# adri-romsor/iterative_inference_segm

Measured on AMD Instinct MI355X. Metric: refined images/s (FCN-8 + standard DAE, 10-step iterative inference, 224x224, 11 classes), higher is better.
Workload: dtype f32; 1 GPU; BASELINE configs[1]: FCN-8 + standard DAE (f64c1p2, pool4, trackind, skip), 224x224x3, batch 64/GPU, 10 steps, step 0.1, early stop off; per batch: pred_fcn_fn, val_fn, pred_dae_fn+val_fn, refine, val_fn; global_batch=64, parallelism=dp1

## Files before the change

include/iiseg.h:

```cpp
#ifndef IISEG_H
#define IISEG_H

#include <stdint.h>

#ifdef __cplusplus
extern "C" {
#endif

typedef enum iiseg_status {
    IISEG_OK = 0,
    IISEG_ERR_NULL = -1,
    IISEG_ERR_SHAPE = -2,
    IISEG_ERR_ALIGN = -3,
    IISEG_ERR_LAUNCH = -4,
    IISEG_ERR_UNSUPPORTED = -5
} iiseg_status;

const char* iiseg_strerror(int status);
const char* iiseg_last_hip_error(void);
int iiseg_abi_version(void);
const char* iiseg_target_arch(void);

int iiseg_profile_begin(int capacity);
int iiseg_profile_count(void);
// ... 40 lines not shown
int iiseg_conv_pool_f32(void* stream, const iiseg_conv_desc* d, const float* x1, const float* x2,
                        const float* pre, const float* pooled, const float* wp, const int32_t* ktab,
                        const float* bias, const float* add, float* out, float* pool_out);

int iiseg_conv_mask_supported(const iiseg_conv_desc* d);
int iiseg_conv_mask_f32(void* stream, const iiseg_conv_desc* d, const float* x1, const float* x2,
                        const float* pre, const float* pooled, const uint8_t* mask_in,
                        const float* wp, const int32_t* ktab, const float* bias, const float* add,
                        float* out, float* pool_out, uint8_t* mask_out);

int iiseg_conv_halo_seam(int on);
int64_t iiseg_conv_halo_seam_launches(void);

int iiseg_conv_bnrelu_supported(const iiseg_conv_desc* d);
int iiseg_conv_bnrelu_f32(void* stream, const iiseg_conv_desc* d, const float* x, int64_t x_bstride,
                          const float* beta, const float* gamma, const float* mean,
                          const float* inv_std, const float* wp, const int32_t* ktab,
                          const float* bias, float* out);

#define IISEG_WINO_INPUT 1u
#define IISEG_WINO_GEMM 2u
#define IISEG_WINO_OUTPUT 4u
#define IISEG_WINO_ALL 7u
#define IISEG_WINO_FUSED 8u
int iiseg_conv_wino_supported(const iiseg_conv_desc* d);
int64_t iiseg_conv_wino_weight_elems(const iiseg_conv_desc* d);
int64_t iiseg_conv_wino_workspace_elems(const iiseg_conv_desc* d);
int iiseg_conv_wino_pack_f32(void* stream, const iiseg_conv_desc* d, const float* w,
                             int64_t stride_o, int64_t stride_c, float* U);
int iiseg_conv_wino_f32(void* stream, const iiseg_conv_desc* d, const float* x1, const float* x2,
                        const float* pre, const float* pooled, const float* U, const float* bias,
                        const float* add, float* workspace, float* out, uint32_t stages);
int iiseg_conv_wino_input_wide(int on);
int iiseg_conv_wino_input_path(const iiseg_conv_desc* d, int mask_bytes);
int iiseg_conv_wino_pool_supported(const iiseg_conv_desc* d);
int iiseg_conv_wino_mask_f32(void* stream, const iiseg_conv_desc* d, const float* x1, const float* x2,
                             const float* pre, const float* pooled, const uint8_t* mask_in,
                             const float* U, const float* bias, const float* add, float* workspace,
                             float* out, float* pool_out, uint8_t* mask_out, uint32_t stages);

int iiseg_conv_wino_bf16_supported(const iiseg_conv_desc* d);
int64_t iiseg_conv_wino_bf16_weight_bytes(const iiseg_conv_desc* d);
int64_t iiseg_conv_wino_bf16_workspace_bytes(const iiseg_conv_desc* d);
int iiseg_conv_wino_bf16_pack(void* stream, const iiseg_conv_desc* d, const float* w,
                              int64_t stride_o, int64_t stride_c, void* U16);
int iiseg_conv_wino_bf16(void* stream, const iiseg_conv_desc* d, const float* x1, const float* x2,
                         const float* pre, const float* pooled, const void* U16, const float* bias,
                         const float* add, void* workspace, float* out, uint32_t stages);

int iiseg_conv_gemm_bf16_supported(const iiseg_conv_desc* d);
int64_t iiseg_conv_gemm_bf16_weight_bytes(const iiseg_conv_desc* d);
int64_t iiseg_conv_gemm_bf16_workspace_bytes(const iiseg_conv_desc* d);
int iiseg_conv_gemm_bf16_pack(void* stream, const iiseg_conv_desc* d, const float* w,
                              int64_t stride_o, int64_t stride_c, void* U16);
int iiseg_conv_gemm_bf16(void* stream, const iiseg_conv_desc* d, const float* x, const void* U16,
                         const float* bias, void* workspace, float* out);

int iiseg_conv_halo_bf16_supported(const iiseg_conv_desc* d);
int64_t iiseg_conv_halo_bf16_weight_bytes(const iiseg_conv_desc* d);
int iiseg_conv_halo_bf16_pack(void* stream, const iiseg_conv_desc* d, const float* w,
                              int64_t stride_o, int64_t stride_c, void* wp16);
int iiseg_conv_halo_bf16(void* stream, const iiseg_conv_desc* d, const float* x1, const float* x2,
                         const float* pre, const float* pooled, const void* wp16, const float* bias,
                         const float* add, float* out, float* pool_out, const uint8_t* mask_in,
                         uint8_t* mask_out);

// ... 336 lines not shown
```

iterative_inference_segm_amd/_lib.py:

```python
import ctypes as C
import os

HERE = os.path.dirname(os.path.abspath(__file__))
LIB_PATH = os.path.join(HERE, 'libiiseg_hip.so')

ABI_VERSION = 34

CONV_RELU = 1
CONV_UNPOOL = 2
CONV_X3 = 8
CONV_TRANSPOSED2 = 4
CONV_ZINS = 16


class ConvDesc(C.Structure):
    _fields_ = [(n, C.c_int32) for n in
                ('B', 'C1', 'C2', 'H', 'W', 'Cout', 'KH', 'KW', 'pad', 'dil',
                 'oy0', 'ox0', 'OH', 'OW', 'AH', 'AW', 'ay0', 'ax0')] + \
               [('flags', C.c_uint32), ('Kpad', C.c_int32), ('Mpad', C.c_int32),
                ('out_ctot', C.c_int32), ('out_c0', C.c_int32),
                ('out_H', C.c_int32), ('out_W', C.c_int32), ('out_y0', C.c_int32),
                ('out_x0', C.c_int32), ('tile_y0', C.c_int32), ('tile_x0', C.c_int32)]


# ... 43 lines not shown


_vp, _i32, _i64, _f32, _f64 = C.c_void_p, C.c_int32, C.c_int64, C.c_float, C.c_double

SIGNATURES = {
    'iiseg_strerror': (C.c_char_p, [C.c_int]),
    'iiseg_last_hip_error': (C.c_char_p, []),
    'iiseg_abi_version': (C.c_int, []),
    'iiseg_profile_begin': (C.c_int, [C.c_int]),
    'iiseg_profile_count': (C.c_int, []),
    'iiseg_profile_end': (C.c_int, [C.POINTER(C.c_float), C.c_int]),
    'iiseg_target_arch': (C.c_char_p, []),
    'iiseg_conv_ktab_entries': (C.c_int, [C.POINTER(ConvDesc)]),
    'iiseg_conv_plan': (C.c_int, [C.POINTER(ConvDesc)]),
    'iiseg_conv_pack_f32': (C.c_int, [_vp, C.POINTER(ConvDesc), _vp, _i64, _i64, _vp, _vp]),
    'iiseg_conv_f32': (C.c_int, [_vp, C.POINTER(ConvDesc)] + [_vp] * 9),
    'iiseg_conv_small_supported': (C.c_int, [C.POINTER(ConvDesc)]),
    'iiseg_conv_pool_supported': (C.c_int, [C.POINTER(ConvDesc)]),
    'iiseg_conv_direct_kernel': (C.c_int, [C.POINTER(ConvDesc), C.c_int, C.c_int, C.POINTER(C.c_int32)]),
    'iiseg_conv_pool_f32': (C.c_int, [_vp, C.POINTER(ConvDesc)] + [_vp] * 10),
    'iiseg_conv_halo_seam': (C.c_int, [C.c_int]),
    'iiseg_conv_halo_seam_launches': (_i64, []),
    'iiseg_conv_mask_supported': (C.c_int, [C.POINTER(ConvDesc)]),
    'iiseg_conv_mask_f32': (C.c_int, [_vp, C.POINTER(ConvDesc)] + [_vp] * 12),
    'iiseg_conv_bnrelu_supported': (C.c_int, [C.POINTER(ConvDesc)]),
    'iiseg_conv_bnrelu_f32': (C.c_int, [_vp, C.POINTER(ConvDesc), _vp, _i64] + [_vp] * 8),
    'iiseg_conv_wino_supported': (C.c_int, [C.POINTER(ConvDesc)]),
    'iiseg_conv_wino_weight_elems': (_i64, [C.POINTER(ConvDesc)]),
    'iiseg_conv_wino_workspace_elems': (_i64, [C.POINTER(ConvDesc)]),
    'iiseg_conv_wino_pack_f32': (C.c_int, [_vp, C.POINTER(ConvDesc), _vp, _i64, _i64, _vp]),
    'iiseg_conv_wino_f32': (C.c_int, [_vp, C.POINTER(ConvDesc)] + [_vp] * 9 + [C.c_uint32]),
    'iiseg_conv_wino_pool_supported': (C.c_int, [C.POINTER(ConvDesc)]),
    'iiseg_conv_wino_input_wide': (C.c_int, [C.c_int]),
    'iiseg_conv_wino_input_path': (C.c_int, [C.POINTER(ConvDesc), C.c_int]),
    'iiseg_conv_wino_mask_f32': (C.c_int, [_vp, C.POINTER(ConvDesc)] + [_vp] * 12 + [C.c_uint32]),
    'iiseg_conv_wino_bf16_supported': (C.c_int, [C.POINTER(ConvDesc)]),
    'iiseg_conv_wino_bf16_weight_bytes': (_i64, [C.POINTER(ConvDesc)]),
    'iiseg_conv_wino_bf16_workspace_bytes': (_i64, [C.POINTER(ConvDesc)]),
    'iiseg_conv_wino_bf16_pack': (C.c_int, [_vp, C.POINTER(ConvDesc), _vp, _i64, _i64, _vp]),
    'iiseg_conv_wino_bf16': (C.c_int, [_vp, C.POINTER(ConvDesc)] + [_vp] * 9 + [C.c_uint32]),
    'iiseg_conv_gemm_bf16_supported': (C.c_int, [C.POINTER(ConvDesc)]),
    'iiseg_conv_gemm_bf16_weight_bytes': (_i64, [C.POINTER(ConvDesc)]),
    'iiseg_conv_gemm_bf16_workspace_bytes': (_i64, [C.POINTER(ConvDesc)]),
    'iiseg_conv_gemm_bf16_pack': (C.c_int, [_vp, C.POINTER(ConvDesc), _vp, _i64, _i64, _vp]),
    'iiseg_conv_gemm_bf16': (C.c_int, [_vp, C.POINTER(ConvDesc)] + [_vp] * 5),
    'iiseg_conv_halo_bf16_supported': (C.c_int, [C.POINTER(ConvDesc)]),
    'iiseg_conv_halo_bf16_weight_bytes': (_i64, [C.POINTER(ConvDesc)]),
    'iiseg_conv_halo_bf16_pack': (C.c_int, [_vp, C.POINTER(ConvDesc), _vp, _i64, _i64, _vp]),
    'iiseg_conv_halo_bf16': (C.c_int, [_vp, C.POINTER(ConvDesc)] + [_vp] * 11),
    'iiseg_conv_wino_f64_supported': (C.c_int, [C.POINTER(ConvDesc)]),
    'iiseg_conv_wino_f64_weight_elems': (_i64, [C.POINTER(ConvDesc)]),
    'iiseg_conv_wino_f64_workspace_elems': (_i64, [C.POINTER(ConvDesc)]),
    'iiseg_conv_wino_pack_f64': (C.c_int, [_vp, C.POINTER(ConvDesc), _vp, _i64, _i64, _vp]),
    'iiseg_conv_wino_f64': (C.c_int, [_vp, C.POINTER(ConvDesc)] + [_vp] * 9),
    'iiseg_conv_c8_supported': (C.c_int, [C.POINTER(ConvDesc)]),
    'iiseg_conv_c8_is_flat': (C.c_int, [C.POINTER(ConvDesc)]),
    'iiseg_conv_c8_force_tiling': (C.c_int, [C.c_int, C.c_int, C.c_int]),
    'iiseg_conv_c8_tiling': (C.c_int, [C.POINTER(ConvDesc), C.c_int, C.POINTER(C.c_int32)]),
    'iiseg_conv_c8': (C.c_int, [_vp, C.POINTER(ConvDesc)] + [_vp] * 6 + [_i32, _vp, _i32, _vp, _vp]),
    'iiseg_conv_c8_slice': (C.c_int, [_vp, C.POINTER(ConvDesc), _vp, _i32] + [_vp] * 5 + [_i32, _vp, _i32, _vp, _vp]),
    'iiseg_unpool_c8': (C.c_int, [_vp] * 4 + [C.c_int] * 7),
    'iiseg_conv_c8_m16_supported': (C.c_int, [C.POINTER(ConvDesc)]),
    'iiseg_conv_c8_m16': (C.c_int, [_vp, C.POINTER(ConvDesc), _vp, _i32] + [_vp] * 6 + [_i32]),
    'iiseg_conv_c8_m16_workspace_bytes': (_i64, [C.POINTER(ConvDesc)]),
    'iiseg_conv_c8_m16_ws': (C.c_int, [_vp, C.POINTER(ConvDesc), _vp, _i32] + [_vp] * 6 + [_i32, _vp, _i64, _vp, _vp, _f64] + [_vp] * 4 + [_i32]),
    'iiseg_conv1x1_c8_weight_bytes': (_i64, [C.c_int, C.c_int]),
# ... 146 lines not shown
```

iterative_inference_segm_amd/csrc/conv_wino.hip:

```cpp
#include <hip/hip_runtime.h>
#include <stdint.h>
#include <stdlib.h>
#include <atomic>
#include <type_traits>
#include "iiseg.h"
#include "common.h"
#include "conv_common.h"

using namespace iiseg;

namespace {

struct WinoParams {
    const float* x1;
    const float* x2;
    const float* pre;
    const float* pooled;
    const uint8_t* mask_in;
    int h2, w2;
    const float* U;
    const float* bias;
    const float* add;
    float* V;
    float* M;
    float* out;
    int B, C1, C2, H, W;
    int Cout, pad;
    int oy0, ox0, OH, OW;
    int ty0, tx0, nty, ntx;
    int T, Tpad;
    int Kc, Mpad;
    int AH, AW, ay0, ax0;
    int relu;
    int out_ctot, out_c0, out_H, out_W, out_y0, out_x0;
    int n_ttiles, n_mtiles;
    float* pool;
    uint8_t* mask_out;
    int pool_H, pool_W;
};

__device__ __forceinline__ float pool4(float v00, float v01, float v10, float v11) {
    const float a = v00 > v01 ? v00 : v01;
    const float b = v10 > v11 ? v10 : v11;
    return a > b ? a : b;
}

__device__ __forceinline__ void pool_store(const WinoParams& p, int b, int co, int ay, int ax,
                                           float v00, float v01, float v10, float v11) {
    const float m = pool4(v00, v01, v10, v11);
    const size_t po = ((size_t)b * p.Cout + co) * p.pool_H * p.pool_W + (size_t)(ay >> 1) * p.pool_W + (ax >> 1);
    p.pool[po] = m;
    if (p.mask_out)
        p.mask_out[po] = (uint8_t)((v00 == m ? 1u : 0u) | (v01 == m ? 2u : 0u) |
                                   (v10 == m ? 4u : 0u) | (v11 == m ? 8u : 0u));
}

constexpr int RSRC_W3 = 0x00027000;

__device__ __forceinline__ __amdgpu_buffer_rsrc_t mk_rsrc(const float* base, int bytes) {
    return __builtin_amdgcn_make_buffer_rsrc((void*)base, 0, bytes, RSRC_W3);
}

__global__ void wino_weight_kernel(const float* __restrict__ w, int64_t so, int64_t sc,
                                   float* __restrict__ U, int Cin, int Cout, int Kc, int Mpad) {
    const int64_t n = (int64_t)Kc * Mpad;
    for (int64_t i = blockIdx.x * (int64_t)blockDim.x + threadIdx.x; i < n;
         i += (int64_t)gridDim.x * blockDim.x) {
        const int c = (int)(i / Mpad), co = (int)(i % Mpad);
        double g[3][3], t[4][3];
        const bool real = c < Cin && co < Cout;
#pragma unroll
        for (int a = 0; a < 3; ++a)
#pragma unroll
            for (int b = 0; b < 3; ++b) g[a][b] = real ? (double)w[co * so + c * sc + a * 3 + b] : 0.0;
#pragma unroll
        for (int b = 0; b < 3; ++b) {
            t[0][b] = g[0][b];
            t[1][b] = 0.5 * (g[0][b] + g[1][b] + g[2][b]);
            t[2][b] = 0.5 * (g[0][b] - g[1][b] + g[2][b]);
            t[3][b] = g[2][b];
        }
#pragma unroll
        for (int a = 0; a < 4; ++a) {
            const double u0 = t[a][0], u1 = 0.5 * (t[a][0] + t[a][1] + t[a][2]),
                         u2 = 0.5 * (t[a][0] - t[a][1] + t[a][2]), u3 = t[a][2];
            U[(int64_t)(a * 4 + 0) * n + i] = (float)u0;
            U[(int64_t)(a * 4 + 1) * n + i] = (float)u1;
            U[(int64_t)(a * 4 + 2) * n + i] = (float)u2;
            U[(int64_t)(a * 4 + 3) * n + i] = (float)u3;
        }
    }
}

constexpr int ICH = 4;
template <bool UNPOOL, int PY, int PX, bool MB = false>
// ... 351 lines not shown
                const float* Lb = L + lbase[j] + RB[i] * NC;
                const float2 alo = *reinterpret_cast<const float2*>(La);
                const float2 ahi = *reinterpret_cast<const float2*>(La + 2);
                const float2 blo = *reinterpret_cast<const float2*>(Lb);
                const float2 bhi = *reinterpret_cast<const float2*>(Lb + 2);
                const float da[4] = {alo.x, alo.y, ahi.x, ahi.y}, db[4] = {blo.x, blo.y, bhi.x, bhi.y};
                float e[4];
#pragma unroll
                for (int jj = 0; jj < 4; ++jj) e[jj] = i == 1 ? da[jj] + db[jj] : da[jj] - db[jj];
                o[0][j] = e[0] - e[2];
                o[1][j] = e[1] + e[2];
                o[2][j] = e[2] - e[1];
                o[3][j] = e[1] - e[3];
            }
            if (FULL || nv == 4) {
#pragma unroll
                for (int x = 0; x < 4; ++x)
                    *reinterpret_cast<float4*>(vo + (size_t)(i * 4 + x) * xis) =
                        make_float4(o[x][0], o[x][1], o[x][2], o[x][3]);
            } else {
#pragma unroll
                for (int x = 0; x < 4; ++x)
#pragma unroll
                    for (int j = 0; j < 3; ++j)
                        if (j < nv) vo[(size_t)(i * 4 + x) * xis + j] = o[x][j];
            }
        }
    }
    };
    if (tw0 + 4 * NT <= p.T) run(std::true_type{});
    else run(std::false_type{});
}

template <int BM, int BN, int WM, int WN, int NBUF, int BK = 16>
__global__ __launch_bounds__(WM * WN * 64, 2) void wino_gemm_kernel(const WinoParams p) {
    constexpr int NCH = BK / 2;
    constexpr int WTM = BM / WM, WTN = BN / WN;
    constexpr int TM = WTM / 32, TN = WTN / 32;
    constexpr int NW = WM * WN, NT = NW * 64;
    constexpr int AV = BK * BM / 4, BV = BK * BN / 4;
    constexpr int NA = NW == 8 ? 256 : NT;
    constexpr int APT = AV / NA, BPT = BV / 256;
    static_assert((NW == 4 || NW == 8) && AV % NA == 0 && BV % 256 == 0, "tile config");

    __shared__ __attribute__((aligned(16))) float As[NBUF][BK][BM];
    __shared__ __attribute__((aligned(16))) float Bs[NBUF][BK][BN];

    const int per_xi = p.n_ttiles * p.n_mtiles;
    int xi, tt, mt;
    {
        const int nb = gridDim.x, bid = blockIdx.x;
        const int q = nb / 8, r = nb % 8, xcd = bid % 8, l = bid / 8;
        const int v = (xcd < r ? xcd * (q + 1) : r * (q + 1) + (xcd - r) * q) + l;
        xi = v / per_xi;
        const int w = v - xi * per_xi;
        constexpr int GP = 8;
        const int gsize = GP * p.n_mtiles;
        const int g = w / gsize, rr = w % gsize;
        const int gp = min(GP, p.n_ttiles - g * GP);
        tt = g * GP + rr % gp;
        mt = rr / gp;
    }
    const int m0 = mt * BM, t0 = tt * BN;
    const int tid = threadIdx.x, lane = tid & 63, wave = tid >> 6;
    const int wm = wave / WN, wn = wave % WN;
    const int l31 = lane & 31, lh = lane >> 5;

    const __amdgpu_buffer_rsrc_t arsrc = mk_rsrc(p.U + (size_t)xi * p.Kc * p.Mpad, p.Kc * p.Mpad * 4);
    const __amdgpu_buffer_rsrc_t brsrc = mk_rsrc(p.V + (size_t)xi * p.Kc * p.Tpad, p.Kc * p.Tpad * 4);
    const bool bstager = NW == 4 || wave < 4;
    const bool astager = NW == 4 || wave >= 4;
    const int atid = NW == 8 ? tid - 256 : tid;
    const int awave = NW == 8 ? wave - 4 : wave;

#define WINO_STAGE(KT, BUF)                                                                        \
    {                                                                                              \
        if (astager)                                                                               \
            static_for<0, APT>([&](auto J) __attribute__((always_inline)) {                        \
                constexpr int j = decltype(J)::value;                                              \
                const int f = j * NA + atid;                                                       \
                const int row = f / (BM / 4), c4 = f % (BM / 4);                                   \
                __builtin_amdgcn_raw_ptr_buffer_load_lds(                                          \
                    arsrc,                                                                         \
                    (__attribute__((address_space(3))) void*)(&As[BUF][0][0] + (j * NA + awave * 64) * 4), \
                    16, (int)(4u * (unsigned)(((KT) * BK + row) * p.Mpad + m0 + c4 * 4)), 0, 0, 0); \
            });                                                                                    \
        if (bstager)                                                                               \
            static_for<0, BPT>([&](auto J) __attribute__((always_inline)) {                        \
                constexpr int j = decltype(J)::value;                                              \
                const int f = j * 256 + (tid & 255);                                               \
                const int row = f / (BN / 4), c4 = f % (BN / 4);                                   \
                __builtin_amdgcn_raw_ptr_buffer_load_lds(                                          \
                    brsrc,                                                                         \
                    (__attribute__((address_space(3))) void*)(&Bs[BUF][0][0] + (j * 256 + (wave & 3) * 64) * 4), \
                    16, (int)(4u * (unsigned)(((KT) * BK + row) * p.Tpad + t0 + c4 * 4)), 0, 0, 0); \
            });                                                                                    \
    }

    f32x16 acc[TM][TN];
#pragma unroll
    for (int i = 0; i < TM; ++i)
#pragma unroll
        for (int j = 0; j < TN; ++j)
#pragma unroll
            for (int r = 0; r < 16; ++r) acc[i][j][r] = 0.f;

    const int nkt = p.Kc / BK;
    constexpr int OPS_A = APT, OPS_B = BPT;
#define WINO_WAIT_ONE_STAGE_IN_FLIGHT()                                                            \
    {                                                                                              \
        if constexpr (NW == 8) {                                                                   \
            if (astager) asm volatile("s_waitcnt vmcnt(%0)" ::"n"(OPS_A) : "memory");              \
            else asm volatile("s_waitcnt vmcnt(%0)" ::"n"(OPS_B) : "memory");                      \
        } else {                                                                                   \
            asm volatile("s_waitcnt vmcnt(%0)" ::"n"(OPS_A + OPS_B) : "memory");                   \
        }                                                                                          \
    }
    WINO_STAGE(0, 0)
    if constexpr (NBUF == 3) {
        if (nkt > 1) {
            WINO_STAGE(1, 1)
            WINO_WAIT_ONE_STAGE_IN_FLIGHT()
        } else {
            asm volatile("s_waitcnt vmcnt(0)" ::: "memory");
        }
    } else {
        asm volatile("s_waitcnt vmcnt(0)" ::: "memory");
    }
    __syncthreads();

    int buf = 0;
    for (int kt = 0; kt < nkt; ++kt) {
        const bool more = kt + NBUF - 1 < nkt;
        int sbuf = buf + NBUF - 1;
        if (sbuf >= NBUF) sbuf -= NBUF;
        float a[2][TM], b[2][TN];
#pragma unroll
        for (int i = 0; i < TM; ++i) a[0][i] = As[buf][lh][wm * WTM + i * 32 + l31];
#pragma unroll
        for (int j = 0; j < TN; ++j) b[0][j] = Bs[buf][lh][wn * WTN + j * 32 + l31];
        static_for<0, NCH>([&](auto CH) __attribute__((always_inline)) {
            constexpr int ch = decltype(CH)::value;
            if constexpr (ch + 1 < NCH) {
                const int kk = (ch + 1) * 2 + lh;
#pragma unroll
                for (int i = 0; i < TM; ++i) a[(ch + 1) & 1][i] = As[buf][kk][wm * WTM + i * 32 + l31];
#pragma unroll
                for (int j = 0; j < TN; ++j) b[(ch + 1) & 1][j] = Bs[buf][kk][wn * WTN + j * 32 + l31];
            }
#pragma unroll
            for (int i = 0; i < TM; ++i)
#pragma unroll
                for (int j = 0; j < TN; ++j)
                    acc[i][j] = __builtin_amdgcn_mfma_f32_32x32x2f32(a[ch & 1][i], b[ch & 1][j],
                                                                     acc[i][j], 0, 0, 0);
            if constexpr (ch == 0) {
                if (more) WINO_STAGE(kt + NBUF - 1, sbuf)
            }
            __builtin_amdgcn_sched_barrier(0);
        });
        if (NBUF == 3 && more) {
            WINO_WAIT_ONE_STAGE_IN_FLIGHT()
        } else {
            asm volatile("s_waitcnt vmcnt(0)" ::: "memory");
        }
        __syncthreads();
        if (++buf == NBUF) buf = 0;
    }
#undef WINO_STAGE
#undef WINO_WAIT_ONE_STAGE_IN_FLIGHT

    float* Mx = p.M + (size_t)xi * p.Mpad * p.Tpad;
#pragma unroll
    for (int j = 0; j < TN; ++j) {
        const int t = t0 + wn * WTN + j * 32 + l31;
#pragma unroll
        for (int i = 0; i < TM; ++i)
#pragma unroll
            for (int r = 0; r < 16; ++r) {
                const int co = m0 + wm * WTM + i * 32 + (r & 3) + 8 * (r >> 2) + 4 * lh;
                Mx[(size_t)co * p.Tpad + t] = acc[i][j][r];
            }
    }
}

template <int BM, int BN, int WM, int WN, int BK, int MINW>
__global__ __launch_bounds__(WM * WN * 64, MINW) void wino_fused_kernel(const WinoParams p) {
    constexpr int NCH = BK / 2;
    constexpr int WTM = BM / WM, WTN = BN / WN;
    constexpr int TM = WTM / 32, TN = WTN / 32;
    constexpr int NT = WM * WN * 64;
    constexpr int AV = BK * BM / 4, BV = BK * BN / 4;
    constexpr int APT = AV / NT, BPT = BV / NT;
    static_assert(AV % NT == 0 && BV % NT == 0, "tile config");

    __shared__ __attribute__((aligned(16))) float As[2][BK][BM];
    __shared__ __attribute__((aligned(16))) float Bs[2][BK][BN];

    int tt, mt;
    tile_of_block(blockIdx.x, gridDim.x, p.n_ttiles, p.n_mtiles, tt, mt);
    const int m0 = mt * BM, t0 = tt * BN;
    const int tid = threadIdx.x, lane = tid & 63, wave = tid >> 6;
    const int wm = wave / WN, wn = wave % WN;
    const int l31 = lane & 31, lh = lane >> 5;
    const int nkt = p.Kc / BK;
    const size_t ustride = (size_t)p.Kc * p.Mpad, vstride = (size_t)p.Kc * p.Tpad;
    const int ubytes = p.Kc * p.Mpad * 4, vbytes = p.Kc * p.Tpad * 4;

#define WINO_STAGE(XI, KT, BUF)                                                                    \
    {                                                                                              \
        const __amdgpu_buffer_rsrc_t ar = mk_rsrc(p.U + (size_t)(XI) * ustride, ubytes);           \
        const __amdgpu_buffer_rsrc_t br = mk_rsrc(p.V + (size_t)(XI) * vstride, vbytes);           \
        static_for<0, APT>([&](auto J) __attribute__((always_inline)) {                            \
            constexpr int j = decltype(J)::value;                                                  \
            const int f = j * NT + tid;                                                            \
            const int row = f / (BM / 4), c4 = f % (BM / 4);                                       \
            __builtin_amdgcn_raw_ptr_buffer_load_lds(                                              \
                ar, (__attribute__((address_space(3))) void*)(&As[BUF][0][0] + (j * NT + wave * 64) * 4), \
                16, (int)(4u * (unsigned)(((KT) * BK + row) * p.Mpad + m0 + c4 * 4)), 0, 0, 0);    \
        });                                                                                        \
        static_for<0, BPT>([&](auto J) __attribute__((always_inline)) {                            \
            constexpr int j = decltype(J)::value;                                                  \
            const int f = j * NT + tid;                                                            \
            const int row = f / (BN / 4), c4 = f % (BN / 4);                                       \
            __builtin_amdgcn_raw_ptr_buffer_load_lds(                                              \
                br, (__attribute__((address_space(3))) void*)(&Bs[BUF][0][0] + (j * NT + wave * 64) * 4), \
                16, (int)(4u * (unsigned)(((KT) * BK + row) * p.Tpad + t0 + c4 * 4)), 0, 0, 0);    \
        });                                                                                        \
    }

    f32x16 acc[TM][TN], Y[4][TM][TN];
#pragma unroll
    for (int i = 0; i < TM; ++i)
#pragma unroll
        for (int j = 0; j < TN; ++j)
#pragma unroll
            for (int r = 0; r < 16; ++r) {
                acc[i][j][r] = 0.f;
                Y[0][i][j][r] = Y[1][i][j][r] = Y[2][i][j][r] = Y[3][i][j][r] = 0.f;
            }

    WINO_STAGE(0, 0, 0)
    asm volatile("s_waitcnt vmcnt(0)" ::: "memory");
    __syncthreads();

    int xi = 0, kt = 0;
    const int total = 16 * nkt;
    for (int s = 0; s < total; ++s) {
        const int buf = s & 1;
        int nxi = xi, nkt1 = kt + 1;
        if (nkt1 == nkt) { nkt1 = 0; ++nxi; }
        const bool more = s + 1 < total;
        float a[2][TM], b[2][TN];
#pragma unroll
        for (int i = 0; i < TM; ++i) a[0][i] = As[buf][lh][wm * WTM + i * 32 + l31];
#pragma unroll
        for (int j = 0; j < TN; ++j) b[0][j] = Bs[buf][lh][wn * WTN + j * 32 + l31];
        static_for<0, NCH>([&](auto CH) __attribute__((always_inline)) {
            constexpr int ch = decltype(CH)::value;
            if constexpr (ch + 1 < NCH) {
                const int kk = (ch + 1) * 2 + lh;
#pragma unroll
                for (int i = 0; i < TM; ++i) a[(ch + 1) & 1][i] = As[buf][kk][wm * WTM + i * 32 + l31];
#pragma unroll
                for (int j = 0; j < TN; ++j) b[(ch + 1) & 1][j] = Bs[buf][kk][wn * WTN + j * 32 + l31];
            }
#pragma unroll
            for (int i = 0; i < TM; ++i)
#pragma unroll
                for (int j = 0; j < TN; ++j)
                    acc[i][j] = __builtin_amdgcn_mfma_f32_32x32x2f32(a[ch & 1][i], b[ch & 1][j],
                                                                     acc[i][j], 0, 0, 0);
            if constexpr (ch == 0) {
                if (more) WINO_STAGE(nxi, nkt1, buf ^ 1)
            }
            __builtin_amdgcn_sched_barrier(0);
        });
        if (nkt1 == 0) {
            const int wi = xi >> 2, wj = xi & 3;
            const float r0 = wi < 3 ? 1.f : 0.f, r1 = wi == 0 ? 0.f : (wi == 1 ? 1.f : -1.f);
            const float c0 = wj < 3 ? 1.f : 0.f, c1 = wj == 0 ? 0.f : (wj == 1 ? 1.f : -1.f);
            const float k00 = r0 * c0, k01 = r0 * c1, k10 = r1 * c0, k11 = r1 * c1;
#define WINO_FOLD(Q, KQ)                                                                            \
            if ((KQ) != 0.f) {                                                                      \
                _Pragma("unroll") for (int i = 0; i < TM; ++i)                                      \
                _Pragma("unroll") for (int j = 0; j < TN; ++j)                                      \
                _Pragma("unroll") for (int r = 0; r < 16; ++r)                                      \
                    Y[Q][i][j][r] = fmaf((KQ), acc[i][j][r], Y[Q][i][j][r]);                        \
            }
            WINO_FOLD(0, k00)
            WINO_FOLD(1, k01)
            WINO_FOLD(2, k10)
            WINO_FOLD(3, k11)
#undef WINO_FOLD
#pragma unroll
            for (int i = 0; i < TM; ++i)
#pragma unroll
                for (int j = 0; j < TN; ++j)
#pragma unroll
                    for (int r = 0; r < 16; ++r) acc[i][j][r] = 0.f;
        }
        xi = nxi;
        kt = nkt1;
        asm volatile("s_waitcnt vmcnt(0)" ::: "memory");
        __syncthreads();
    }
#undef WINO_STAGE

    typedef float f32x2u __attribute__((ext_vector_type(2), aligned(4)));
    const int ntt = p.nty * p.ntx;
    const size_t OPL = (size_t)p.out_H * p.out_W, APL = (size_t)p.AH * p.AW;
    float* Lbias = &As[0][0][0];
    for (int f = tid; f < BM; f += NT) Lbias[f] = (p.bias && m0 + f < p.Cout) ? p.bias[m0 + f] : 0.f;
    __syncthreads();
    float bias_r[TM][16];
#pragma unroll
    for (int i = 0; i < TM; ++i)
#pragma unroll
        for (int r = 0; r < 16; ++r) bias_r[i][r] = Lbias[wm * WTM + i * 32 + (r & 3) + 8 * (r >> 2) + 4 * lh];
#pragma unroll
    for (int j = 0; j < TN; ++j) {
        const int t = t0 + wn * WTN + j * 32 + l31;
        if (t >= p.T) continue;
        const int b = t / ntt;
        const int rr = t - b * ntt;
        const int tyl = rr / p.ntx, txl = rr - tyl * p.ntx;
        const int wy = p.ty0 + 2 * tyl - p.oy0, wx = p.tx0 + 2 * txl - p.ox0;
        const bool rok[2] = {(unsigned)wy < (unsigned)p.OH, (unsigned)(wy + 1) < (unsigned)p.OH};
        const bool cok[2] = {(unsigned)wx < (unsigned)p.OW, (unsigned)(wx + 1) < (unsigned)p.OW};
        const bool pair = cok[0] && cok[1];
        const bool whole = p.pool && rok[1] && cok[1];
        float* ob = p.out ? p.out + ((size_t)b * p.out_ctot + p.out_c0) * OPL +
                                (ptrdiff_t)(p.out_y0 + wy) * p.out_W + p.out_x0 + wx
                          : nullptr;
        const float* ab = p.add ? p.add + (size_t)b * p.Cout * APL +
                                      (ptrdiff_t)(p.ay0 + wy) * p.AW + p.ax0 + wx
                                : nullptr;
#pragma unroll
        for (int i = 0; i < TM; ++i)
#pragma unroll
            for (int r = 0; r < 16; ++r) {
                const int co = m0 + wm * WTM + i * 32 + (r & 3) + 8 * (r >> 2) + 4 * lh;
                if (co >= p.Cout) continue;
                const float bias = bias_r[i][r];
// ... 134 lines not shown
        d->pad < 0 || d->OH <= 0 || d->OW <= 0 || d->oy0 < 0 || d->ox0 < 0)
        return IISEG_ERR_SHAPE;
    const int fullH = d->H + 2 * d->pad - 2, fullW = d->W + 2 * d->pad - 2;
    if (d->oy0 + d->OH > fullH || d->ox0 + d->OW > fullW) return IISEG_ERR_SHAPE;
    if ((d->C1 + d->C2) % 16) return IISEG_ERR_UNSUPPORTED;
    g.Kc = d->C1 + d->C2;
    g.bm = d->Cout > 128 ? 256 : (d->Cout > 64 ? 128 : 64);
    g.Mpad = round_up(d->Cout, g.bm);
    if ((d->tile_y0 | d->tile_x0) & ~1) return IISEG_ERR_SHAPE;
    g.ty0 = d->oy0 - ((d->oy0 - d->tile_y0) & 1);
    g.tx0 = d->ox0 - ((d->ox0 - d->tile_x0) & 1);
    g.nty = (d->oy0 + d->OH - g.ty0 + 1) >> 1;
    g.ntx = (d->ox0 + d->OW - g.tx0 + 1) >> 1;
    const int64_t T = (int64_t)d->B * g.nty * g.ntx;
    const int64_t Tpad = (T + 127) / 128 * 128;
    if (Tpad * g.Kc * 4 >= (int64_t)1 << 31 || (int64_t)g.Kc * g.Mpad * 4 >= (int64_t)1 << 31)
        return IISEG_ERR_UNSUPPORTED;
    g.T = (int)T;
    g.Tpad = (int)Tpad;
    return IISEG_OK;
}

std::atomic<int> g_input_wide{-1};

int input_wide_setting() {
    int v = g_input_wide.load();
    if (v < 0) {
        v = getenv("IISEG_WINO_INPUT_WIDE") ? (atoi(getenv("IISEG_WINO_INPUT_WIDE")) != 0) : 1;
        g_input_wide.store(v);
    }
    return v;
}

bool iw_fits(const WinoParams& p, int nt) {
    const int NC = 2 * p.ntx + 2;
    for (int t0 = 0; t0 < p.T; t0 += 4 * nt) {
        const int t1 = t0 + 4 * nt < p.T ? t0 + 4 * nt : p.T;
        if ((int64_t)iw_chunk(t0, t1, p.ntx, p.nty).NR * NC > (int64_t)IW_E * nt) return false;
    }
    return true;
}

int ilds_nt(const WinoParams& p);
constexpr int IW_NT = 256;

int iw_shape(const WinoParams& p, bool unpool, bool mb) {
    const int setting = input_wide_setting();
    if (!setting || (unpool && !mb)) return 0;
    if (setting != 2) {
        if (p.T < 4096) return 0;
        const int lnt = mb ? 0 : ilds_nt(p);
        if (lnt && (p.nty * p.ntx) % lnt == 0) return 0;
    }
    const int64_t HW = (int64_t)p.H * p.W, cmax = p.C1 > p.C2 ? p.C1 : p.C2;
    if (HW > (1 << IW_PBITS) || (int64_t)p.B * cmax * HW >= (int64_t)1 << 30) return 0;
    const int64_t waves1 = ((int64_t)p.T + 255) / 256 * p.Kc;
    int ch = 8;
    if (p.Kc % 32 == 0 && waves1 / 32 >= 2048) ch = 32;
    else if (waves1 / 16 >= 2048) ch = 16;
    return iw_fits(p, IW_NT) ? ch : 0;
}

int ilds_nt(const WinoParams& p) {
    static const int lds = getenv("IISEG_WINO_INPUT_LDS") ? atoi(getenv("IISEG_WINO_INPUT_LDS")) : 1;
    const int ntt = p.nty * p.ntx;
    int nt = 0;
// ... 54 lines not shown
                             int Tpad, const float* bias, const float* add, float* out) {
    WinoParams p = {};
    p.M = const_cast<float*>(M);
    p.bias = bias; p.add = add; p.out = out;
    p.B = d->B; p.Cout = d->Cout; p.pad = d->pad;
    p.oy0 = d->oy0; p.ox0 = d->ox0; p.OH = d->OH; p.OW = d->OW;
    p.ty0 = d->oy0 - ((d->oy0 - d->tile_y0) & 1);
    p.tx0 = d->ox0 - ((d->ox0 - d->tile_x0) & 1);
    p.nty = (d->oy0 + d->OH - p.ty0 + 1) >> 1;
    p.ntx = (d->ox0 + d->OW - p.tx0 + 1) >> 1;
    p.T = d->B * p.nty * p.ntx;
    p.Tpad = Tpad; p.Mpad = Mpad;
    p.AH = d->AH; p.AW = d->AW; p.ay0 = d->ay0; p.ax0 = d->ax0;
    p.relu = (d->flags & IISEG_CONV_RELU) ? 1 : 0;
    p.out_ctot = d->out_ctot > 0 ? d->out_ctot : d->Cout;
    p.out_c0 = d->out_ctot > 0 ? d->out_c0 : 0;
    p.out_H = d->out_H > 0 ? d->out_H : d->OH;
    p.out_W = d->out_H > 0 ? d->out_W : d->OW;
    p.out_y0 = d->out_H > 0 ? d->out_y0 : 0;
    p.out_x0 = d->out_H > 0 ? d->out_x0 : 0;
    IISEG_LAUNCH(wino_output_kernel, dim3((p.T + 255) / 256, (d->Cout + OCH - 1) / OCH),
                       dim3(256), 0, s, p);
    return iiseg_check_launch();
}

extern "C" int iiseg_conv_wino_supported(const iiseg_conv_desc* d) {
    WinoGeom g;
    return wino_geom(d, g) == IISEG_OK ? 1 : 0;
}

extern "C" int iiseg_conv_wino_input_wide(int on) {
    if (on >= 0) g_input_wide.store(on > 1 ? 2 : on);
    return input_wide_setting();
}

extern "C" int iiseg_conv_wino_input_path(const iiseg_conv_desc* d, int mask_bytes) {
    WinoGeom g;
    const int st = wino_geom(d, g);
    if (st) return st;
    WinoParams p = {};
    const bool unpool = (d->flags & IISEG_CONV_UNPOOL) != 0;
    if (mask_bytes && !unpool) return IISEG_ERR_UNSUPPORTED;
    p.B = d->B; p.C1 = d->C1; p.C2 = d->C2; p.H = d->H; p.W = d->W;
    p.nty = g.nty; p.ntx = g.ntx; p.T = g.T; p.Tpad = g.Tpad; p.Kc = g.Kc;
    if (iw_shape(p, unpool, mask_bytes != 0)) return 2;
    return ilds_nt(p) ? 1 : 0;
}

extern "C" int64_t iiseg_conv_wino_weight_elems(const iiseg_conv_desc* d) {
    WinoGeom g;
    if (wino_geom(d, g) != IISEG_OK) return 0;
    return (int64_t)16 * g.Kc * g.Mpad;
}

extern "C" int64_t iiseg_conv_wino_workspace_elems(const iiseg_conv_desc* d) {
    WinoGeom g;
    if (wino_geom(d, g) != IISEG_OK) return 0;
    return (int64_t)16 * g.Tpad * ((int64_t)g.Kc + g.Mpad);
}

extern "C" int iiseg_conv_wino_pack_f32(void* stream, const iiseg_conv_desc* d, const float* w,
                                        int64_t stride_o, int64_t stride_c, float* U) {
    WinoGeom g;
    const int st = wino_geom(d, g);
    if (st) return st;
    if (!w || !U) return IISEG_ERR_NULL;
// ... 48 lines not shown
    p.U = U;
    p.bias = bias;
    p.add = add;
    p.V = workspace;
    p.M = workspace + (size_t)16 * g.Kc * g.Tpad;
    p.out = out;
    p.B = d->B; p.C1 = d->C1; p.C2 = d->C2; p.H = d->H; p.W = d->W;
    p.Cout = d->Cout; p.pad = d->pad;
    p.oy0 = d->oy0; p.ox0 = d->ox0; p.OH = d->OH; p.OW = d->OW;
    p.ty0 = g.ty0; p.tx0 = g.tx0; p.nty = g.nty; p.ntx = g.ntx;
    p.T = g.T; p.Tpad = g.Tpad; p.Kc = g.Kc; p.Mpad = g.Mpad;
    p.AH = d->AH; p.AW = d->AW; p.ay0 = d->ay0; p.ax0 = d->ax0;
    if (add && (d->ay0 < 0 || d->ax0 < 0 || d->ay0 + d->OH > d->AH || d->ax0 + d->OW > d->AW))
        return IISEG_ERR_SHAPE;
    p.relu = (d->flags & IISEG_CONV_RELU) ? 1 : 0;
    p.out_ctot = d->out_ctot > 0 ? d->out_ctot : d->Cout;
    p.out_c0 = d->out_ctot > 0 ? d->out_c0 : 0;
    if (p.out_c0 < 0 || p.out_c0 + d->Cout > p.out_ctot) return IISEG_ERR_SHAPE;
    p.out_H = d->out_H > 0 ? d->out_H : d->OH;
    p.out_W = d->out_H > 0 ? d->out_W : d->OW;
    p.out_y0 = d->out_H > 0 ? d->out_y0 : 0;
    p.out_x0 = d->out_H > 0 ? d->out_x0 : 0;
    if (p.out_y0 < 0 || p.out_x0 < 0 || p.out_y0 + d->OH > p.out_H || p.out_x0 + d->OW > p.out_W)
        return IISEG_ERR_SHAPE;
    p.n_ttiles = g.Tpad / 128;
    p.n_mtiles = g.Mpad / g.bm;
    hipStream_t s = (hipStream_t)stream;
    const int tb = (g.T + 255) / 256;
    if (stages & IISEG_WINO_FUSED) {
        if (g.Kc % 32) return IISEG_ERR_UNSUPPORTED;
        if (stages & IISEG_WINO_INPUT)
            launch_wino_input(s, p, unpool);
        if (stages & IISEG_WINO_GEMM) {
            if (g.bm == 64) {
                p.n_mtiles = g.Mpad / 64;
                IISEG_LAUNCH((wino_fused_kernel<64, 128, 1, 4, 32, 2>),
                                   dim3(p.n_ttiles * p.n_mtiles), dim3(256), 0, s, p);
                return iiseg_check_launch();
            }
            p.n_mtiles = g.Mpad / 128;
            const int w0 = p.n_ttiles * p.n_mtiles, w2 = (g.Tpad / 64) * p.n_mtiles;
            const double cost0 = (w0 + 255) / 256, cost2 = 0.5 * 1.03 * ((w2 + 255) / 256);
            static const int bk64 = getenv("IISEG_WINO_FUSED_BK") ? atoi(getenv("IISEG_WINO_FUSED_BK")) == 64 : 0;
            const bool big = bk64 && g.Kc % 64 == 0;
            if (g.Kc <= 128 || cost2 < cost0) {
                p.n_ttiles = g.Tpad / 64;
                if (big)
                    IISEG_LAUNCH((wino_fused_kernel<128, 64, 2, 2, 64, 2>),
                                       dim3(p.n_ttiles * p.n_mtiles), dim3(256), 0, s, p);
                else
                IISEG_LAUNCH((wino_fused_kernel<128, 64, 2, 2, 32, 2>),
                                   dim3(p.n_ttiles * p.n_mtiles), dim3(256), 0, s, p);
            } else if (big)
                IISEG_LAUNCH((wino_fused_kernel<128, 128, 2, 4, 64, 2>),
                                   dim3(p.n_ttiles * p.n_mtiles), dim3(512), 0, s, p);
            else
            IISEG_LAUNCH((wino_fused_kernel<128, 128, 2, 4, 32, 2>),
                               dim3(p.n_ttiles * p.n_mtiles), dim3(512), 0, s, p);
        }
        return iiseg_check_launch();
    }
    if (stages & IISEG_WINO_INPUT)
        launch_wino_input(s, p, unpool);
    const int grid = 16 * p.n_ttiles * p.n_mtiles;
    if (stages & IISEG_WINO_GEMM) {
        static const int nbuf = getenv("IISEG_WINO_NBUF") ? atoi(getenv("IISEG_WINO_NBUF")) : 2;
        int bm = g.bm;
        if (bm == 64) {
            IISEG_LAUNCH((wino_gemm_kernel<64, 128, 1, 4, 2>), dim3(grid), dim3(256), 0, s, p);
            bm = 0;
        }
        if (bm == 256) {
            const int w256 = grid, w128 = 2 * grid;
            if (0.5 * 1.06 * ((w128 + 255) / 256) < (double)((w256 + 255) / 256)) bm = 128;
        }
        const int grid2 = bm ? 16 * p.n_ttiles * (g.Mpad / bm) : 0;
        if (bm) p.n_mtiles = g.Mpad / bm;
        static const int bk32 = getenv("IISEG_WINO_GEMM_BK") ? atoi(getenv("IISEG_WINO_GEMM_BK")) == 32 : 0;
        if (bm && bk32 && g.Kc % 32 == 0 && nbuf != 3) {
            if (bm == 256)
                IISEG_LAUNCH((wino_gemm_kernel<256, 128, 4, 2, 2, 32>), dim3(grid), dim3(512), 0, s, p);
            else
                IISEG_LAUNCH((wino_gemm_kernel<128, 128, 2, 2, 2, 32>), dim3(grid2), dim3(256), 0, s, p);
        } else
        if (bm == 0) {
        } else if (bm == 256 && nbuf == 3)
            IISEG_LAUNCH((wino_gemm_kernel<256, 128, 4, 2, 3>), dim3(grid), dim3(512), 0, s, p);
        else if (bm == 256)
            IISEG_LAUNCH((wino_gemm_kernel<256, 128, 4, 2, 2>), dim3(grid), dim3(512), 0, s, p);
        else if (nbuf == 3)
            IISEG_LAUNCH((wino_gemm_kernel<128, 128, 2, 2, 3>), dim3(grid2), dim3(256), 0, s, p);
        else
            IISEG_LAUNCH((wino_gemm_kernel<128, 128, 2, 2, 2>), dim3(grid2), dim3(256), 0, s, p);
    }
    if (stages & IISEG_WINO_OUTPUT)
        IISEG_LAUNCH(wino_output_kernel, dim3(tb, (d->Cout + OCH - 1) / OCH), dim3(256), 0, s,
                           p);
    return iiseg_check_launch();
}

extern "C" int iiseg_conv_wino_f32(void* stream, const iiseg_conv_desc* d, const float* x1,
                                   const float* x2, const float* pre, const float* pooled,
                                   const float* U, const float* bias,
                                   const float* add, float* workspace, float* out,
                                   uint32_t stages) {
    return wino_run(stream, d, x1, x2, pre, pooled, nullptr, U, bias, add, workspace, out, nullptr,
                    nullptr, stages);
}

extern "C" int iiseg_conv_wino_mask_f32(void* stream, const iiseg_conv_desc* d, const float* x1,
                                        const float* x2, const float* pre, const float* pooled,
                                        const uint8_t* mask_in, const float* U, const float* bias,
// ... 148 lines not shown
```

Baseline: 536.1 images/s.

## Add configurable three-deep LDS ring to fused Winograd GEMM with inline-asm DMA

Replaces the builtin buffer-load-to-LDS calls with inline-asm buffer_load_dwordx4 ... lds using precomputed per-thread offsets and scalar k-offsets, and swaps __syncthreads for raw s_barrier. Adds an optional 3-buffer ring to the fused Winograd kernel, with partial vmcnt waits so that two stages can be in flight. Ring depth is selectable via env or API, but defaults stay at 2, so by default only the address and barrier rewrite takes effect. The hand-written m0 manipulation and raw barriers risk ordering bugs and add extra register pressure.

Result: no change. 541.0 images/s, median of 6 (+0.9%).

```diff
diff --git a/include/iiseg.h b/include/iiseg.h
--- a/include/iiseg.h
+++ b/include/iiseg.h
@@ -96,6 +96,7 @@
                         const float* pre, const float* pooled, const float* U, const float* bias,
                         const float* add, float* workspace, float* out, uint32_t stages);
 int iiseg_conv_wino_input_wide(int on);
+int iiseg_conv_wino_ring_depth(int fused, int depth);
 int iiseg_conv_wino_input_path(const iiseg_conv_desc* d, int mask_bytes);
 int iiseg_conv_wino_pool_supported(const iiseg_conv_desc* d);
 int iiseg_conv_wino_mask_f32(void* stream, const iiseg_conv_desc* d, const float* x1, const float* x2,
diff --git a/iterative_inference_segm_amd/_lib.py b/iterative_inference_segm_amd/_lib.py
--- a/iterative_inference_segm_amd/_lib.py
+++ b/iterative_inference_segm_amd/_lib.py
@@ -99,6 +99,7 @@
     'iiseg_conv_wino_f32': (C.c_int, [_vp, C.POINTER(ConvDesc)] + [_vp] * 9 + [C.c_uint32]),
     'iiseg_conv_wino_pool_supported': (C.c_int, [C.POINTER(ConvDesc)]),
     'iiseg_conv_wino_input_wide': (C.c_int, [C.c_int]),
+    'iiseg_conv_wino_ring_depth': (C.c_int, [C.c_int, C.c_int]),
     'iiseg_conv_wino_input_path': (C.c_int, [C.POINTER(ConvDesc), C.c_int]),
     'iiseg_conv_wino_mask_f32': (C.c_int, [_vp, C.POINTER(ConvDesc)] + [_vp] * 12 + [C.c_uint32]),
     'iiseg_conv_wino_bf16_supported': (C.c_int, [C.POINTER(ConvDesc)]),
diff --git a/iterative_inference_segm_amd/csrc/conv_wino.hip b/iterative_inference_segm_amd/csrc/conv_wino.hip
--- a/iterative_inference_segm_amd/csrc/conv_wino.hip
+++ b/iterative_inference_segm_amd/csrc/conv_wino.hip
@@ -55,12 +55,6 @@
                                    (v10 == m ? 4u : 0u) | (v11 == m ? 8u : 0u));
 }
 
-constexpr int RSRC_W3 = 0x00027000;
-
-__device__ __forceinline__ __amdgpu_buffer_rsrc_t mk_rsrc(const float* base, int bytes) {
-    return __builtin_amdgcn_make_buffer_rsrc((void*)base, 0, bytes, RSRC_W3);
-}
-
 __global__ void wino_weight_kernel(const float* __restrict__ w, int64_t so, int64_t sc,
                                    float* __restrict__ U, int Cin, int Cout, int Kc, int Mpad) {
     const int64_t n = (int64_t)Kc * Mpad;
@@ -478,6 +472,17 @@
     else run(std::false_type{});
 }
 
+__device__ __forceinline__ void ring_barrier() { asm volatile("s_barrier" ::: "memory"); }
+
+__device__ __forceinline__ void ring_dma16(i32x4s rsrc, unsigned lds, unsigned voff, unsigned soff) {
+    unsigned keep;
+    asm volatile("s_nop 1\n\ts_mov_b32 %0, m0\n\ts_mov_b32 m0, %1\n\ts_nop 0\n\t"
+                 "buffer_load_dwordx4 %2, %3, %4 offen lds\n\ts_mov_b32 m0, %0"
+                 : "=&s"(keep)
+                 : "s"(lds), "v"(voff), "s"(rsrc), "s"(soff)
+                 : "memory");
+}
+
 template <int BM, int BN, int WM, int WN, int NBUF, int BK = 16>
 __global__ __launch_bounds__(WM * WN * 64, 2) void wino_gemm_kernel(const WinoParams p) {
     constexpr int NCH = BK / 2;
@@ -512,35 +517,44 @@
     const int wm = wave / WN, wn = wave % WN;
     const int l31 = lane & 31, lh = lane >> 5;
 
-    const __amdgpu_buffer_rsrc_t arsrc = mk_rsrc(p.U + (size_t)xi * p.Kc * p.Mpad, p.Kc * p.Mpad * 4);
-    const __amdgpu_buffer_rsrc_t brsrc = mk_rsrc(p.V + (size_t)xi * p.Kc * p.Tpad, p.Kc * p.Tpad * 4);
+    const i32x4s arsrc = mk_srsrc(p.U + (size_t)xi * p.Kc * p.Mpad, (unsigned)(p.Kc * p.Mpad * 4));
+    const i32x4s brsrc = mk_srsrc(p.V + (size_t)xi * p.Kc * p.Tpad, (unsigned)(p.Kc * p.Tpad * 4));
     const bool bstager = NW == 4 || wave < 4;
     const bool astager = NW == 4 || wave >= 4;
-    const int atid = NW == 8 ? tid - 256 : tid;
-    const int awave = NW == 8 ? wave - 4 : wave;
-
+    const int atid = NW == 8 ? (tid & 255) : tid;
+    const int awave = NW == 8 ? (wave & 3) : wave;
+
+    unsigned aoff[APT], boff[BPT];
+#pragma unroll
+    for (int j = 0; j < APT; ++j) {
+        const int f = j * NA + atid;
+        const int row = f / (BM / 4), c4 = f % (BM / 4);
+        aoff[j] = 4u * (unsigned)(row * p.Mpad + m0 + c4 * 4);
+    }
+#pragma unroll
+    for (int j = 0; j < BPT; ++j) {
+        const int f = j * 256 + (tid & 255);
+        const int row = f / (BN / 4), c4 = f % (BN / 4);
+        boff[j] = 4u * (unsigned)(row * p.Tpad + t0 + c4 * 4);
+    }
+    const unsigned a_lds = __builtin_amdgcn_readfirstlane(lds_addr(&As[0][0][0]) + (unsigned)awave * 1024u);
+    const unsigned b_lds = __builtin_amdgcn_readfirstlane(lds_addr(&Bs[0][0][0]) + (unsigned)(wave & 3) * 1024u);
 #define WINO_STAGE(KT, BUF)                                                                        \
     {                                                                                              \
-        if (astager)                                                                               \
+        if (astager) {                                                                             \
+            const unsigned so = __builtin_amdgcn_readfirstlane(4u * (unsigned)((KT) * BK * p.Mpad)); \
             static_for<0, APT>([&](auto J) __attribute__((always_inline)) {                        \
                 constexpr int j = decltype(J)::value;                                              \
-                const int f = j * NA + atid;                                                       \
-                const int row = f / (BM / 4), c4 = f % (BM / 4);                                   \
-                __builtin_amdgcn_raw_ptr_buffer_load_lds(                                          \
-                    arsrc,                                                                         \
-                    (__attribute__((address_space(3))) void*)(&As[BUF][0][0] + (j * NA + awave * 64) * 4), \
-                    16, (int)(4u * (unsigned)(((KT) * BK + row) * p.Mpad + m0 + c4 * 4)), 0, 0, 0); \
+                ring_dma16(arsrc, a_lds + (unsigned)(BUF) * (BK * BM * 4u) + j * NA * 16u, aoff[j], so); \
             });                                                                                    \
-        if (bstager)                                                                               \
+        }                                                                                          \
+        if (bstager) {                                                                             \
+            const unsigned so = __builtin_amdgcn_readfirstlane(4u * (unsigned)((KT) * BK * p.Tpad)); \
             static_for<0, BPT>([&](auto J) __attribute__((always_inline)) {                        \
                 constexpr int j = decltype(J)::value;                                              \
-                const int f = j * 256 + (tid & 255);                                               \
-                const int row = f / (BN / 4), c4 = f % (BN / 4);                                   \
-                __builtin_amdgcn_raw_ptr_buffer_load_lds(                                          \
-                    brsrc,                                                                         \
-                    (__attribute__((address_space(3))) void*)(&Bs[BUF][0][0] + (j * 256 + (wave & 3) * 64) * 4), \
-                    16, (int)(4u * (unsigned)(((KT) * BK + row) * p.Tpad + t0 + c4 * 4)), 0, 0, 0); \
+                ring_dma16(brsrc, b_lds + (unsigned)(BUF) * (BK * BN * 4u) + j * 256 * 16u, boff[j], so); \
             });                                                                                    \
+        }                                                                                          \
     }
 
     f32x16 acc[TM][TN];
@@ -573,7 +587,7 @@
     } else {
         asm volatile("s_waitcnt vmcnt(0)" ::: "memory");
     }
-    __syncthreads();
+    ring_barrier();
 
     int buf = 0;
     for (int kt = 0; kt < nkt; ++kt) {
@@ -610,7 +624,8 @@
         } else {
             asm volatile("s_waitcnt vmcnt(0)" ::: "memory");
         }
-        __syncthreads();
+        ring_barrier();
+        __builtin_amdgcn_sched_barrier(0);
         if (++buf == NBUF) buf = 0;
     }
 #undef WINO_STAGE
@@ -630,7 +645,7 @@
     }
 }
 
-template <int BM, int BN, int WM, int WN, int BK, int MINW>
+template <int BM, int BN, int WM, int WN, int BK, int MINW, int NBUF = 2>
 __global__ __launch_bounds__(WM * WN * 64, MINW) void wino_fused_kernel(const WinoParams p) {
     constexpr int NCH = BK / 2;
     constexpr int WTM = BM / WM, WTN = BN / WN;
@@ -639,9 +654,10 @@
     constexpr int AV = BK * BM / 4, BV = BK * BN / 4;
     constexpr int APT = AV / NT, BPT = BV / NT;
     static_assert(AV % NT == 0 && BV % NT == 0, "tile config");
-
-    __shared__ __attribute__((aligned(16))) float As[2][BK][BM];
-    __shared__ __attribute__((aligned(16))) float Bs[2][BK][BN];
+    static_assert(NBUF == 2 || NBUF == 3, "ring depth");
+
+    __shared__ __attribute__((aligned(16))) float As[NBUF][BK][BM];
+    __shared__ __attribute__((aligned(16))) float Bs[NBUF][BK][BN];
 
     int tt, mt;
     tile_of_block(blockIdx.x, gridDim.x, p.n_ttiles, p.n_mtiles, tt, mt);
@@ -653,25 +669,34 @@
     const size_t ustride = (size_t)p.Kc * p.Mpad, vstride = (size_t)p.Kc * p.Tpad;
     const int ubytes = p.Kc * p.Mpad * 4, vbytes = p.Kc * p.Tpad * 4;
 
+    unsigned aoff[APT], boff[BPT];
+#pragma unroll
+    for (int j = 0; j < APT; ++j) {
+        const int f = j * NT + tid;
+        const int row = f / (BM / 4), c4 = f % (BM / 4);
+        aoff[j] = 4u * (unsigned)(row * p.Mpad + m0 + c4 * 4);
+    }
+#pragma unroll
+    for (int j = 0; j < BPT; ++j) {
+        const int f = j * NT + tid;
+        const int row = f / (BN / 4), c4 = f % (BN / 4);
+        boff[j] = 4u * (unsigned)(row * p.Tpad + t0 + c4 * 4);
+    }
+    const unsigned a_lds = __builtin_amdgcn_readfirstlane(lds_addr(&As[0][0][0]) + (unsigned)wave * 1024u);
+    const unsigned b_lds = __builtin_amdgcn_readfirstlane(lds_addr(&Bs[0][0][0]) + (unsigned)wave * 1024u);
 #define WINO_STAGE(XI, KT, BUF)                                                                    \
     {                                                                                              \
-        const __amdgpu_buffer_rsrc_t ar = mk_rsrc(p.U + (size_t)(XI) * ustride, ubytes);           \
-        const __amdgpu_buffer_rsrc_t br = mk_rsrc(p.V + (size_t)(XI) * vstride, vbytes);           \
+        const i32x4s ar = mk_srsrc(p.U + (size_t)(XI) * ustride, (unsigned)ubytes);                \
+        const i32x4s br = mk_srsrc(p.V + (size_t)(XI) * vstride, (unsigned)vbytes);                \
+        const unsigned soa = __builtin_amdgcn_readfirstlane(4u * (unsigned)((KT) * BK * p.Mpad));  \
+        const unsigned sob = __builtin_amdgcn_readfirstlane(4u * (unsigned)((KT) * BK * p.Tpad));  \
         static_for<0, APT>([&](auto J) __attribute__((always_inline)) {                            \
             constexpr int j = decltype(J)::value;                                                  \
-            const int f = j * NT + tid;                                                            \
-            const int row = f / (BM / 4), c4 = f % (BM / 4);                                       \
-            __builtin_amdgcn_raw_ptr_buffer_load_lds(                                              \
-                ar, (__attribute__((address_space(3))) void*)(&As[BUF][0][0] + (j * NT + wave * 64) * 4), \
-                16, (int)(4u * (unsigned)(((KT) * BK + row) * p.Mpad + m0 + c4 * 4)), 0, 0, 0);    \
+            ring_dma16(ar, a_lds + (unsigned)(BUF) * (BK * BM * 4u) + j * NT * 16u, aoff[j], soa); \
         });                                                                                        \
         static_for<0, BPT>([&](auto J) __attribute__((always_inline)) {                            \
             constexpr int j = decltype(J)::value;                                                  \
-            const int f = j * NT + tid;                                                            \
-            const int row = f / (BN / 4), c4 = f % (BN / 4);                                       \
-            __builtin_amdgcn_raw_ptr_buffer_load_lds(                                              \
-                br, (__attribute__((address_space(3))) void*)(&Bs[BUF][0][0] + (j * NT + wave * 64) * 4), \
-                16, (int)(4u * (unsigned)(((KT) * BK + row) * p.Tpad + t0 + c4 * 4)), 0, 0, 0);    \
+            ring_dma16(br, b_lds + (unsigned)(BUF) * (BK * BN * 4u) + j * NT * 16u, boff[j], sob); \
         });                                                                                        \
     }
 
@@ -686,17 +711,28 @@
                 Y[0][i][j][r] = Y[1][i][j][r] = Y[2][i][j][r] = Y[3][i][j][r] = 0.f;
             }
 
+    constexpr int OPS = APT + BPT;
+    const int total = 16 * nkt;
+    int sxi = 0, skt = 0;
     WINO_STAGE(0, 0, 0)
-    asm volatile("s_waitcnt vmcnt(0)" ::: "memory");
-    __syncthreads();
+    if (++skt == nkt) { skt = 0; ++sxi; }
+    if constexpr (NBUF == 3) {
+        WINO_STAGE(sxi, skt, 1)
+        if (++skt == nkt) { skt = 0; ++sxi; }
+        asm volatile("s_waitcnt vmcnt(%0)" ::"n"(OPS) : "memory");
+    } else {
+        asm volatile("s_waitcnt vmcnt(0)" ::: "memory");
+    }
+    ring_barrier();
 
     int xi = 0, kt = 0;
-    const int total = 16 * nkt;
+    int buf = 0;
     for (int s = 0; s < total; ++s) {
-        const int buf = s & 1;
-        int nxi = xi, nkt1 = kt + 1;
-        if (nkt1 == nkt) { nkt1 = 0; ++nxi; }
-        const bool more = s + 1 < total;
+        int nkt1 = kt + 1;
+        if (nkt1 == nkt) nkt1 = 0;
+        const bool more = s + NBUF - 1 < total;
+        int sbuf = buf + NBUF - 1;
+        if (sbuf >= NBUF) sbuf -= NBUF;
         float a[2][TM], b[2][TN];
 #pragma unroll
         for (int i = 0; i < TM; ++i) a[0][i] = As[buf][lh][wm * WTM + i * 32 + l31];
@@ -718,10 +754,11 @@
                     acc[i][j] = __builtin_amdgcn_mfma_f32_32x32x2f32(a[ch & 1][i], b[ch & 1][j],
                                                                      acc[i][j], 0, 0, 0);
             if constexpr (ch == 0) {
-                if (more) WINO_STAGE(nxi, nkt1, buf ^ 1)
+                if (more) WINO_STAGE(sxi, skt, sbuf)
             }
             __builtin_amdgcn_sched_barrier(0);
         });
+        if (more && ++skt == nkt) { skt = 0; ++sxi; }
         if (nkt1 == 0) {
             const int wi = xi >> 2, wj = xi & 3;
             const float r0 = wi < 3 ? 1.f : 0.f, r1 = wi == 0 ? 0.f : (wi == 1 ? 1.f : -1.f);
@@ -746,16 +783,25 @@
 #pragma unroll
                     for (int r = 0; r < 16; ++r) acc[i][j][r] = 0.f;
         }
-        xi = nxi;
+        if (nkt1 == 0) ++xi;
         kt = nkt1;
-        asm volatile("s_waitcnt vmcnt(0)" ::: "memory");
-        __syncthreads();
+        __builtin_amdgcn_sched_barrier(0);
+        if (NBUF == 3 && more) {
+            asm volatile("s_waitcnt vmcnt(%0)" ::"n"(OPS) : "memory");
+        } else {
+            asm volatile("s_waitcnt vmcnt(0)" ::: "memory");
+        }
+        ring_barrier();
+        __builtin_amdgcn_sched_barrier(0);
+        if (++buf == NBUF) buf = 0;
     }
 #undef WINO_STAGE
 
     typedef float f32x2u __attribute__((ext_vector_type(2), aligned(4)));
     const int ntt = p.nty * p.ntx;
     const size_t OPL = (size_t)p.out_H * p.out_W, APL = (size_t)p.AH * p.AW;
+    asm volatile("s_waitcnt vmcnt(0)" ::: "memory");
+    __syncthreads();
     float* Lbias = &As[0][0][0];
     for (int f = tid; f < BM; f += NT) Lbias[f] = (p.bias && m0 + f < p.Cout) ? p.bias[m0 + f] : 0.f;
     __syncthreads();
@@ -956,6 +1002,20 @@
     return v;
 }
 
+std::atomic<int> g_ring_depth[2] = {{-1}, {-1}};
+constexpr int WINO_GEMM_NBUF_256 = 2, WINO_GEMM_NBUF_128 = 2, WINO_FUSED_NBUF = 2;
+
+int ring_depth_setting(int fused) {
+    int v = g_ring_depth[fused].load();
+    if (v < 0) {
+        const char* e = getenv(fused ? "IISEG_WINO_FUSED_NBUF" : "IISEG_WINO_NBUF");
+        v = e ? atoi(e) : 0;
+        if (v != 2 && v != 3) v = 0;
+        g_ring_depth[fused].store(v);
+    }
+    return v;
+}
+
 bool iw_fits(const WinoParams& p, int nt) {
     const int NC = 2 * p.ntx + 2;
     for (int t0 = 0; t0 < p.T; t0 += 4 * nt) {
@@ -1076,6 +1136,12 @@
 extern "C" int iiseg_conv_wino_input_wide(int on) {
     if (on >= 0) g_input_wide.store(on > 1 ? 2 : on);
     return input_wide_setting();
+}
+
+extern "C" int iiseg_conv_wino_ring_depth(int fused, int depth) {
+    const int k = fused ? 1 : 0;
+    if (depth == 0 || depth == 2 || depth == 3) g_ring_depth[k].store(depth);
+    return ring_depth_setting(k);
 }
 
 extern "C" int iiseg_conv_wino_input_path(const iiseg_conv_desc* d, int mask_bytes) {
@@ -1190,10 +1256,16 @@
         if (stages & IISEG_WINO_INPUT)
             launch_wino_input(s, p, unpool);
         if (stages & IISEG_WINO_GEMM) {
+            const int rd = ring_depth_setting(1);
+            const bool ring3 = (rd ? rd : WINO_FUSED_NBUF) == 3;
             if (g.bm == 64) {
                 p.n_mtiles = g.Mpad / 64;
-                IISEG_LAUNCH((wino_fused_kernel<64, 128, 1, 4, 32, 2>),
-                                   dim3(p.n_ttiles * p.n_mtiles), dim3(256), 0, s, p);
+                if (ring3)
+                    IISEG_LAUNCH((wino_fused_kernel<64, 128, 1, 4, 32, 2, 3>),
+                                       dim3(p.n_ttiles * p.n_mtiles), dim3(256), 0, s, p);
+                else
+                    IISEG_LAUNCH((wino_fused_kernel<64, 128, 1, 4, 32, 2>),
+                                       dim3(p.n_ttiles * p.n_mtiles), dim3(256), 0, s, p);
                 return iiseg_check_launch();
             }
             p.n_mtiles = g.Mpad / 128;
@@ -1206,6 +1278,9 @@
                 if (big)
                     IISEG_LAUNCH((wino_fused_kernel<128, 64, 2, 2, 64, 2>),
                                        dim3(p.n_ttiles * p.n_mtiles), dim3(256), 0, s, p);
+                else if (ring3)
+                    IISEG_LAUNCH((wino_fused_kernel<128, 64, 2, 2, 32, 2, 3>),
+                                       dim3(p.n_ttiles * p.n_mtiles), dim3(256), 0, s, p);
                 else
                 IISEG_LAUNCH((wino_fused_kernel<128, 64, 2, 2, 32, 2>),
                                    dim3(p.n_ttiles * p.n_mtiles), dim3(256), 0, s, p);
@@ -1222,7 +1297,7 @@
         launch_wino_input(s, p, unpool);
     const int grid = 16 * p.n_ttiles * p.n_mtiles;
     if (stages & IISEG_WINO_GEMM) {
-        static const int nbuf = getenv("IISEG_WINO_NBUF") ? atoi(getenv("IISEG_WINO_NBUF")) : 2;
+        const int rd = ring_depth_setting(0);
         int bm = g.bm;
         if (bm == 64) {
             IISEG_LAUNCH((wino_gemm_kernel<64, 128, 1, 4, 2>), dim3(grid), dim3(256), 0, s, p);
@@ -1234,8 +1309,9 @@
         }
         const int grid2 = bm ? 16 * p.n_ttiles * (g.Mpad / bm) : 0;
         if (bm) p.n_mtiles = g.Mpad / bm;
+        const int nbuf = rd ? rd : (bm == 256 ? WINO_GEMM_NBUF_256 : WINO_GEMM_NBUF_128);
         static const int bk32 = getenv("IISEG_WINO_GEMM_BK") ? atoi(getenv("IISEG_WINO_GEMM_BK")) == 32 : 0;
-        if (bm && bk32 && g.Kc % 32 == 0 && nbuf != 3) {
+        if (bm && bk32 && g.Kc % 32 == 0 && rd != 3) {
             if (bm == 256)
                 IISEG_LAUNCH((wino_gemm_kernel<256, 128, 4, 2, 2, 32>), dim3(grid), dim3(512), 0, s, p);
             else
```
